# jeya-maria-jose/Medical-Transformer

Measured on AMD Instinct MI355X. Metric: training images/sec (MedT, 3x128x128), higher is better.
Workload: dtype f32; 1 GPU; MedT imgsize=128 bs=4/GPU train step (fwd+CE+bwd+Adam), BASELINE.json configs[2] (per GPU: also configs[3]'s shard); global_batch=4, parallelism=dp1

## Files before the change

medical-transformer_amd/csrc/conv.hip:

```cpp
#include "defer.h"
#include <type_traits>

namespace medt {

template <int K, int OT>
__device__ __forceinline__ void conv2d_fwd_body(
    const float* __restrict__ x, const float* __restrict__ w, const float* __restrict__ bias, float* __restrict__ y,
    float* __restrict__ partials, int Cin, int H, int W, int Cout, int Ho, int Wo, int stride, int pad, int relu,
    int npg, int y_bf16, float* red, int bx, int by) {
    constexpr int KK = K * K;
    const int HoWo = Ho * Wo, per_group = npg * HoWo, ppg = (per_group + MEDT_THREADS - 1) / MEDT_THREADS;
    const int grp = bx / ppg, part = bx - grp * ppg, o0 = by * OT;
    const int q = part * MEDT_THREADS + threadIdx.x;
    const bool ok = q < per_group;
    const int ni = ok ? q / HoWo : 0, p = ok ? q - ni * HoWo : 0;
    const int n = grp * npg + ni;
    const int ho = p / Wo, wo = p - ho * Wo;
    const int h0 = ho * stride - pad, w0 = wo * stride - pad;
    float acc[OT];
#pragma unroll
    for (int o = 0; o < OT; ++o) acc[o] = bias ? bias[o0 + o] : 0.f;
    const float* xn = x + (size_t)n * Cin * H * W;
    int off[KK];
#pragma unroll
// ... 676 lines not shown
            rb[i] = b;
        }
    };
    if (q_begin < q_end) fetch(q_begin);
    for (long q0 = q_begin; q0 < q_end; q0 += 64) {
#pragma unroll
        for (int i = 0; i < NA; ++i) A[r0 + 4 * i][j] = ra[i];
#pragma unroll
        for (int i = 0; i < NB; ++i) B[r0 + 4 * i][j] = rb[i];
        __syncthreads();
        if (q0 + 64 < q_end) fetch(q0 + 64);
#pragma unroll 2
        for (int jj = 0; jj < 64; jj += 4) {
            float4 av[RO], bv[RC];
#pragma unroll
            for (int a = 0; a < RO; ++a) av[a] = *reinterpret_cast<const float4*>(&A[to + 16 * a][jj]);
#pragma unroll
            for (int b = 0; b < RC; ++b) bv[b] = *reinterpret_cast<const float4*>(&B[tc + 16 * b][jj]);
#pragma unroll
            for (int a = 0; a < RO; ++a)
#pragma unroll
                for (int b = 0; b < RC; ++b) {
                    float t = acc[a][b];
                    t = fmaf(av[a].x, bv[b].x, t);
                    t = fmaf(av[a].y, bv[b].y, t);
                    t = fmaf(av[a].z, bv[b].z, t);
                    t = fmaf(av[a].w, bv[b].w, t);
                    acc[a][b] = t;
                }
        }
        __syncthreads();
    }
    float* out = scratch + (size_t)bz * Cout * Ktot;
#pragma unroll
    for (int a = 0; a < RO; ++a)
#pragma unroll
        for (int b = 0; b < RC; ++b) {
            const int o = o0 + to + 16 * a, k = k0 + tc + 16 * b;
            if (o < Cout && k < Ktot) out[(size_t)o * Ktot + k] = acc[a][b];
        }
}

template <int K, int TO, int TC>
__global__ __launch_bounds__(MEDT_THREADS) void conv_wgrad_kernel(
    const float* __restrict__ dy, const float* __restrict__ raw, const float* __restrict__ coef,
    const float* __restrict__ x, float* __restrict__ scratch, int N, int Cin, int H, int W, int Cout, int Ho, int Wo,
    int stride, int pad, int QS, int npg) {
    conv_wgrad_body<K, TO, TC>(dy, raw, coef, x, scratch, N, Cin, H, W, Cout, Ho, Wo, stride, pad, QS, npg, blockIdx.x,
                               blockIdx.y, blockIdx.z);
}

static inline int wgrad_tile(int n) { return n <= 16 ? 16 : (n <= 32 ? 32 : 64); }

static int wgrad_chunk(int Cout, int Ktot, long NP) {
    const long tiles = (long)cdiv(Cout, wgrad_tile(Cout)) * cdiv(Ktot, wgrad_tile(Ktot));
    int QS = 512;
    while (QS > 64 && tiles * ((NP + QS - 1) / QS) < 512) QS >>= 1;
    while ((NP + QS - 1) / QS > 64) QS <<= 1;
    return QS;
}

static int wgrad_chunk_grouped(long NP) {
    static const int target = 64;
    static const int qmax = 256;
    int QS = 64;
    while (QS < qmax && (NP + QS - 1) / QS > target) QS <<= 1;
    static const int smax = 64;
    static const int smax_big = 256;
    while ((NP + QS - 1) / QS > (NP >= 65536 ? smax_big : smax)) QS <<= 1;
    return QS;
}

static int wgrad_chunk_v4(long NP) {
    static const int target = 16;
    static const int qmax = 1024;
    static const int smax_big = 256;
    int QS = 256;
    while (QS < qmax && (NP + QS - 1) / QS > (NP >= 65536 ? smax_big : target)) QS <<= 1;
    while ((NP + QS - 1) / QS > (NP >= 65536 ? smax_big : 64)) QS <<= 1;
    const int QG = wgrad_chunk_grouped(NP);
    return QS > QG ? QS : QG;
}

int conv2d_bwd_weight_splits(int N, int Cin, int Cout, int K, int Ho, int Wo) {
    const long NP = (long)N * Ho * Wo;
    const int QS = wgrad_chunk(Cout, Cin * K * K, NP), QG = wgrad_chunk_grouped(NP);
    const int a = (int)((NP + QS - 1) / QS), b = (int)((NP + QG - 1) / QG);
    return a > b ? a : b;
}

int conv2d_bwd_weight(const float* dy, const float* raw, const float* coef, const float* x, float* dw, float* scratch,
                      int N, int Cin, int H, int W, int Cout, int K, int stride, int pad, int groups, hipStream_t s,
                      Queue* q) {
    const int Ho = (H + 2 * pad - K) / stride + 1, Wo = (W + 2 * pad - K) / stride + 1;
    const long NP = (long)N * Ho * Wo;
    const int Ktot = Cin * K * K;
    const bool mfma = conv_use_mfma(Cin, Cout, K, stride, NP) && Cout >= 64;
    const bool v4 = q && !mfma && conv_wgrad_v4_ok(dy, raw, x, N, Cin, H, W, Cout, Ho, Wo, K, stride, pad);
    const int QS = v4 ? wgrad_chunk_v4(NP) : ((q && !mfma) ? wgrad_chunk_grouped(NP) : wgrad_chunk(Cout, Ktot, NP));
    const int splits = (int)((NP + QS - 1) / QS);
    const dim3 grid(cdiv(Cout, 64), cdiv(Ktot, 64), splits), block(MEDT_THREADS);
    if (splits == 1) scratch = dw;
    if (mfma) {
        static const bool defer_m = true;
        if (q && defer_m) {
            q->mwgrad.push_back(MJob{dy, raw, coef, x, scratch, N, Cin, H, W, Cout, Ho, Wo, K, stride, pad, QS, splits, N / groups});
            if (splits > 1) q->reduce.push_back(RJob{scratch, dw, splits, Cout * Ktot});
            return MEDT_OK;
        }
        int rc = conv_wgrad_mfma(dy, raw, coef, x, scratch, N, Cin, H, W, Cout, Ho, Wo, K, stride, pad, QS, splits,
                                 N / groups, s);
        if (rc) return rc;
        if (splits == 1) return MEDT_OK;
        if (q) { q->reduce.push_back(RJob{scratch, dw, splits, Cout * Ktot}); return MEDT_OK; }
        return reduce_rows(scratch, splits, Cout * Ktot, dw, s);
    }
    if (q) {
        if (K != 1 && K != 3 && K != 7) { set_error("conv2d: kernel size %d unsupported (1, 3, 7)", K); return MEDT_EUNSUPPORTED; }
        q->wgrad.push_back(WJob{dy, raw, coef, x, scratch, N, Cin, H, W, Cout, Ho, Wo, stride, pad, QS, N / groups,
                                cdiv(Cout, 64), cdiv(Ktot, 64), splits, K, v4 ? 1 : 0});
        if (splits > 1) q->reduce.push_back(RJob{scratch, dw, splits, Cout * Ktot});
        return MEDT_OK;
    }
    {
        const int TO = wgrad_tile(Cout), TC = wgrad_tile(Ktot);
        const dim3 g2(cdiv(Cout, TO), cdiv(Ktot, TC), splits);
#define MEDT_WG(KV, TOV, TCV)                                                                                        \
    hipLaunchKernelGGL((conv_wgrad_kernel<KV, TOV, TCV>), g2, block, 0, s, dy, raw, coef, x, scratch, N, Cin, H, W, Cout, Ho, \
                       Wo, stride, pad, QS, N / groups)
#define MEDT_WG_TC(KV, TOV)                                                                                          \
    do { if (TC == 16) MEDT_WG(KV, TOV, 16); else if (TC == 32) MEDT_WG(KV, TOV, 32); else MEDT_WG(KV, TOV, 64); } while (0)
#define MEDT_WG_TO(KV)                                                                                               \
    do { if (TO == 16) MEDT_WG_TC(KV, 16); else if (TO == 32) MEDT_WG_TC(KV, 32); else MEDT_WG_TC(KV, 64); } while (0)
        switch (K) {
            case 1: MEDT_WG_TO(1); break;
            case 3: MEDT_WG_TO(3); break;
            case 7: MEDT_WG_TO(7); break;
            default: set_error("conv2d: kernel size %d unsupported (1, 3, 7)", K); return MEDT_EUNSUPPORTED;
        }
#undef MEDT_WG_TO
#undef MEDT_WG_TC
#undef MEDT_WG
    }
    int rc = launch_status("conv_wgrad");
    if (rc) return rc;
    return splits == 1 ? MEDT_OK : reduce_rows(scratch, splits, Cout * Ktot, dw, s);
}

#define CS_SPLITS 16
int channel_sum_splits_for(int N, int HW) {
    const long total = (long)N * HW;
    long sp = (total + 4095) / 4096;
    return sp < 1 ? 1 : (sp > CS_SPLITS ? CS_SPLITS : (int)sp);
}
__device__ __forceinline__ void channel_sum_body(const float* __restrict__ x, float* __restrict__ part, int N, int C,
                                                 int HW, int c, int sp, int splits) {
    MEDT_STATIC_SHARED float red[MEDT_WAVES];
    float v[1] = {0.f};
    const long total = (long)N * HW;
    const long per = (total + splits - 1) / splits, beg = sp * per, end = beg + per < total ? beg + per : total;
    if (total < (1l << 31)) {
        const unsigned e32 = (unsigned)end, hw = (unsigned)HW;
        float a4[4] = {0.f, 0.f, 0.f, 0.f};
        for (unsigned q = (unsigned)beg + threadIdx.x; q < e32; q += 4 * MEDT_THREADS) {
            float t[4];
#pragma unroll
            for (int u = 0; u < 4; ++u) {
                const unsigned qq = min(q + u * MEDT_THREADS, e32 - 1), n = qq / hw, p = qq - n * hw;
                t[u] = x[((size_t)n * C + c) * HW + p];
            }
#pragma unroll
            for (int u = 0; u < 4; ++u)
                if (q + u * MEDT_THREADS < e32) a4[u] += t[u];
        }
        v[0] = (a4[0] + a4[1]) + (a4[2] + a4[3]);
    } else {
        for (long q = beg + threadIdx.x; q < end; q += MEDT_THREADS) {
            const int n = (int)(q / HW), p = (int)(q - (long)n * HW);
            v[0] += x[((size_t)n * C + c) * HW + p];
        }
    }
    block_sum<1>(v, red, part + (size_t)sp * C + c);
}

__global__ __launch_bounds__(MEDT_THREADS) void channel_sum_kernel(const float* __restrict__ x, float* __restrict__ part,
                                                                   int N, int C, int HW) {
// ... 38 lines not shown
```

medical-transformer_amd/csrc/conv_mfma.hip:

```cpp
#include "defer.h"
#include <algorithm>
#include <vector>
#include <stdlib.h>
#include <stdio.h>

namespace medt {

typedef medt_f4 f32x4;

bool conv_use_mfma(int Cin, int Cout, int K, int stride, long positions) {
    static const bool off = [] { const char* e = getenv("MEDT_DISABLE_MFMA"); return e && e[0] == '1'; }();
    static const bool force = false;
    if (force && !off) return (K == 1 || K == 3) && (stride == 1 || stride == 2);
    const long tiles = ((positions + 63) / 64) * ((Cout + 63) / 64);
    if (off || Cout < 32 || Cin * K * K < 256 || (stride != 1 && stride != 2)) return false;
    if (K == 3 && tiles >= 128) return true;
    static const long few_pos = 2048L;
    return (K == 3 || K == 1) && tiles < 128 && positions <= few_pos && Cin * K * K >= 512;
}

int conv_mfma_parts_per_group(int N, int groups, int HoWo) { return cdiv((N / groups) * HoWo, 64); }

template <int K>
__global__ __launch_bounds__(MEDT_THREADS) void conv_mfma_fwd_kernel(
// ... 627 lines not shown
            if (o < Cout) {
                const float bo = a.bias ? a.bias[o] : 0.f;
                const size_t e0 = ((size_t)n * Cout + o) * HW + (size_t)row0 * W + col;
#pragma unroll
                for (int t = 0; t < TR; ++t) {
                    float v = acc[rb][t][r] + bo;
                    if (a.add) v += a.add[e0 + (size_t)t * W];
                    s1[r] += v;
                    s2[r] = fmaf(v, v, s2[r]);
                    a.y[e0 + (size_t)t * W] = a.relu ? fmaxf(v, 0.f) : v;
                }
            }
        }
        if (a.partials) {
#pragma unroll
            for (int r = 0; r < 4; ++r) {
                double pa = s1[r], pb = s2[r];
#pragma unroll
                for (int m = 8; m > 0; m >>= 1) { pa += __shfl_xor(pa, m, 64); pb += __shfl_xor(pb, m, 64); }
                if ((lane & 15) == 0) {
                    double* d = Rd + ((wv * NRB + rb) * 16 + (lane >> 4) * 4 + r) * 2;
                    d[0] = pa; d[1] = pb;
                }
            }
        }
    }
    if (a.partials) {
        __syncthreads();
        if (kg == 0 && tid < 16 * NRB) {
            const int o = o0 + tid;
            if (o < Cout) {
                double sa = 0.0, sb = 0.0;
#pragma unroll
                for (int w4 = 0; w4 < 4; ++w4) { sa += Rd[(w4 * 16 * NRB + tid) * 2]; sb += Rd[(w4 * 16 * NRB + tid) * 2 + 1]; }
                double* dst = reinterpret_cast<double*>(a.partials) + ((size_t)blockIdx.x * Cout + o) * 2;
                dst[0] = sa;
                dst[1] = sb;
            }
        }
    }
}

int conv_thin_fwd(const float* x, const float* w, const float* bias, const float* add, float* y, float* partials, int N, int groups,
                  int Cin, int H, int W, int Cout, int relu, hipStream_t s) {
    const ThinPlan p = conv_thin_plan(N, groups, Cin, H, W, Cout, 3, 1, 1);
    if (!p.ok) { set_error("conv_thin_fwd: shape not supported"); return MEDT_EUNSUPPORTED; }
    if (abl_skip("conv_thin")) return MEDT_OK;
    ThinArgs a;
    a.x = x; a.w = w; a.bias = bias; a.add = add; a.y = y; a.partials = partials;
    a.Cin = Cin; a.H = H; a.W = W; a.Cout = Cout; a.relu = relu;
    a.TCW = p.TCW; a.RG = p.RG; a.RST = p.RST; a.CST = p.CST; a.PR = p.rows_wg + 2; a.PC = p.cols_wg + 2; a.cwg = W / p.cols_wg;
    a.m_pc = (unsigned)(0x100000000ull / (unsigned)a.PC) + 1u;
    a.m_prpc = (unsigned)(0x100000000ull / (unsigned)(a.PR * a.PC)) + 1u;
    const dim3 grid((unsigned)(N * p.wgs_img), (unsigned)p.grid_y), block(MEDT_THREADS * p.KG);
#define MEDT_THIN(CCv, NRBv, TRv, KGv) hipLaunchKernelGGL((conv3x3_thin_fwd_kernel<CCv, NRBv, TRv, KGv>), grid, block, p.lds, s, a)
#define MEDT_THIN_TR(CCv, NRBv)                         \
    do {                                                \
        if (p.TR == 4) MEDT_THIN(CCv, NRBv, 4, 1);      \
        else if (p.TR == 2) MEDT_THIN(CCv, NRBv, 2, 1); \
        else MEDT_THIN(CCv, NRBv, 1, 1);                \
    } while (0)
    if (p.KG > 1) {
        static unsigned char attr[4][64];
        int rc;
        if ((rc = lds_opt_in((const void*)conv3x3_thin_fwd_kernel<16, 1, 1, 4>, attr[0], "conv3x3_thin_fwd")) ||
            (rc = lds_opt_in((const void*)conv3x3_thin_fwd_kernel<16, 2, 1, 4>, attr[1], "conv3x3_thin_fwd")) ||
            (rc = lds_opt_in((const void*)conv3x3_thin_fwd_kernel<16, 1, 1, 2>, attr[2], "conv3x3_thin_fwd")) ||
            (rc = lds_opt_in((const void*)conv3x3_thin_fwd_kernel<16, 2, 1, 2>, attr[3], "conv3x3_thin_fwd"))) return rc;
        if (p.NRB == 2) { if (p.KG == 4) MEDT_THIN(16, 2, 1, 4); else MEDT_THIN(16, 2, 1, 2); }
        else { if (p.KG == 4) MEDT_THIN(16, 1, 1, 4); else MEDT_THIN(16, 1, 1, 2); }
    }
    else if (p.CC == 16 && p.NRB == 2) MEDT_THIN_TR(16, 2);
    else if (p.CC == 16) MEDT_THIN_TR(16, 1);
    else if (p.NRB == 2) MEDT_THIN_TR(8, 2);
    else MEDT_THIN_TR(8, 1);
#undef MEDT_THIN_TR
#undef MEDT_THIN
    return launch_status("conv3x3_thin_fwd");
}

struct R16WJob {
    const float *dy, *raw, *coef, *x;
    float* scratch;
    int Cin, H, Cout, tiles_per_split, ptiles, npg, gx, gy, gz;
};

template <int OT>
__device__ __forceinline__ void conv3x3_rows16_wgrad_body(const R16WJob& jb, int bx, int by, int bz, float* Ds, float* Ps) {
    constexpr int NR = OT / 4;
    constexpr int NA = OT == 64 ? 9 : 5;
    const float* __restrict__ dy = jb.dy;
    const float* __restrict__ raw = jb.raw;
    const float* __restrict__ coef = jb.coef;
    const float* __restrict__ x = jb.x;
    float* __restrict__ scratch = jb.scratch;
    const int Cin = jb.Cin, H = jb.H, Cout = jb.Cout, tiles_per_split = jb.tiles_per_split, ptiles = jb.ptiles, npg = jb.npg;
    const int tid = threadIdx.x, lane = tid & 63, wv = __builtin_amdgcn_readfirstlane(tid >> 6);
    const int rb = OT == 64 ? wv : (wv & 1), tlo = OT == 64 ? 0 : 5 * (wv >> 1);
    const int o0 = bx * OT, c0 = by * 16;
    const int Ktot = Cin * 9, HW = H * 16, tpi = H >> 2;
    const int pt_begin = bz * tiles_per_split;
    const int pt_end = min(ptiles, pt_begin + tiles_per_split);
    if (tid < 192) {
        const int c = tid / 12, rem = tid - c * 12;
        Ps[c * R16_WCST + (rem >> 1) * R16_RST + (rem & 1) * 17] = 0.f;
    }
    int poff[6], pc[6], prw[6];
#pragma unroll
    for (int i = 0; i < 6; ++i) {
        const int u = tid + MEDT_THREADS * i, c = u / 96, rem = u - c * 96, row = rem >> 4, col = rem & 15;
        poff[i] = c * R16_WCST + row * R16_RST + 1 + col;
        pc[i] = (c0 + c) * HW + col;
        prw[i] = row - 1;
    }
    float rd[NR], rp[6];
    auto fetch = [&](int pt) {
        const int n = pt / tpi, r0 = (pt - n * tpi) * 4;
        const size_t base = (size_t)n * Cout * HW + r0 * 16 + lane;
        const float* cf = coef ? coef + (size_t)(n / npg) * Cout * 3 : nullptr;
#pragma unroll
        for (int j = 0; j < NR; ++j)
            rd[j] = dy[base + (size_t)min(o0 + wv + 4 * j, Cout - 1) * HW];
        if (cf) {
#pragma unroll
            for (int j = 0; j < NR; ++j) {
                const int o = min(o0 + wv + 4 * j, Cout - 1);
                rd[j] = fmaf(cf[o * 3], rd[j], fmaf(cf[o * 3 + 1], raw[base + (size_t)o * HW], cf[o * 3 + 2]));
            }
        }
        const float* xn = x + (size_t)n * Cin * HW;
#pragma unroll
        for (int i = 0; i < 6; ++i) {
            const int gr = r0 + prw[i];
            const float v = xn[pc[i] + min(max(gr, 0), H - 1) * 16];
            rp[i] = (unsigned)gr < (unsigned)H ? v : 0.f;
        }
    };
    f32x4 acc[NA];
#pragma unroll
    for (int t = 0; t < NA; ++t) acc[t] = (f32x4)(0.f);
    int tapoff[NA];
    float tapon[NA];
#pragma unroll
    for (int tt = 0; tt < NA; ++tt) {
        const int t = min(tlo + tt, 8);
        tapoff[tt] = (t / 3) * R16_RST + t % 3;
        tapon[tt] = tlo + tt <= 8 ? 1.f : 0.f;
    }
    const float* drow = Ds + (16 * rb + (lane & 15)) * R16_DST + (lane >> 4);
    const float* prow = Ps + (lane & 15) * R16_WCST + (lane >> 4);
    if (pt_begin < pt_end) fetch(pt_begin);
    for (int pt = pt_begin; pt < pt_end; ++pt) {
#pragma unroll
        for (int j = 0; j < NR; ++j) Ds[(wv + 4 * j) * R16_DST + lane] = rd[j];
#pragma unroll
        for (int i = 0; i < 6; ++i) Ps[poff[i]] = rp[i];
        __syncthreads();
        if (pt + 1 < pt_end) fetch(pt + 1);
#pragma unroll
        for (int ks = 0; ks < 16; ++ks) {
            const float a = drow[ks * 4];
            const float* pk = prow + (ks >> 2) * R16_RST + (ks & 3) * 4;
#pragma unroll
            for (int tt = 0; tt < NA; ++tt)
                acc[tt] = __builtin_amdgcn_mfma_f32_16x16x4f32(OT == 64 ? a : a * tapon[tt], pk[tapoff[tt]], acc[tt], 0, 0, 0);
        }
        __syncthreads();
    }
    float* out = scratch + (size_t)bz * Cout * Ktot;
#pragma unroll
    for (int r = 0; r < 4; ++r) {
        const int o = o0 + 16 * rb + (lane >> 4) * 4 + r;
        if (o < Cout) {
            float* dst = out + (size_t)o * Ktot + (c0 + (lane & 15)) * 9;
#pragma unroll
            for (int tt = 0; tt < NA; ++tt)
                if (tlo + tt <= 8) dst[tlo + tt] = acc[tt][r];
        }
    }
}

using R16WBatch = JobBatch<R16WJob, 4>;
template <int OT>
__global__ __launch_bounds__(MEDT_THREADS) void conv3x3_rows16_wgrad_kernel(R16WBatch b) {
    MEDT_STATIC_SHARED float Ds[OT * R16_DST];
    MEDT_STATIC_SHARED float Ps[16 * R16_WCST];
    const int j = find_job(b, blockIdx.x);
    const R16WJob& jb = b.job[j];
    const int r = blockIdx.x - b.start[j], bx = r % jb.gx, by = (r / jb.gx) % jb.gy, bz = r / (jb.gx * jb.gy);
    conv3x3_rows16_wgrad_body<OT>(jb, bx, by, bz, Ds, Ps);
}

__global__ __launch_bounds__(MEDT_THREADS) void conv_splitk_epilogue_kernel(
    const float* __restrict__ slices, int nslices, size_t slice_stride, const float* __restrict__ bias,
    float* __restrict__ y, float* __restrict__ partials, int Cout, int HoWo, int npg, int ppg64, int relu) {
    MEDT_STATIC_SHARED float red[MEDT_WAVES * 2 * 2];
    const int per_group = npg * HoWo, ppg = (per_group + MEDT_THREADS - 1) / MEDT_THREADS;
    const int grp = blockIdx.x / ppg, part = blockIdx.x - grp * ppg, o = blockIdx.y;
    const int q = part * MEDT_THREADS + threadIdx.x;
    float v[2] = {0.f, 0.f};
    if (q < per_group) {
        const size_t qg = (size_t)grp * ppg64 * 64 + q;
        float a = bias ? bias[o] : 0.f;
        const float* sp = slices + qg * Cout + o;
        int s = 0;
        for (; s + 8 <= nslices; s += 8) {
            float v[8];
#pragma unroll
            for (int u = 0; u < 8; ++u) v[u] = sp[(size_t)(s + u) * slice_stride];
            MEDT_SCHED_FENCE();
#pragma unroll
            for (int u = 0; u < 8; ++u) a += v[u];
            MEDT_SCHED_FENCE();
        }
        for (; s < nslices; ++s) a += sp[(size_t)s * slice_stride];
        const int n = grp * npg + q / HoWo, p = q % HoWo;
        y[((size_t)n * Cout + o) * HoWo + p] = relu ? fmaxf(a, 0.f) : a;
        v[0] = a;
        v[1] = a * a;
    }
    if (partials) block_sum_d<2>(v, red, reinterpret_cast<double*>(partials) + ((size_t)blockIdx.x * Cout + o) * 2);
}

int conv_mfma_ksplit(int Ktot, long tiles, bool rows16) {
#ifdef MEDT_AB_KSPLIT128
    if (tiles >= 128) return 1;
#else
    if (tiles >= 256 || (rows16 && tiles >= 128)) return 1;
    if (tiles >= 128) return Ktot >= 256 ? 2 : 1;
#endif
    int ks = (int)(256 / tiles);
    const int maxks = Ktot / 64 > 0 ? Ktot / 64 : 1;
    if (ks > maxks) ks = maxks;
    return ks < 1 ? 1 : ks;
}

size_t conv_mfma_scratch_floats(int N, int groups, int HoWo, int Cin, int Cout, int K, bool rows16) {
    const long qt = (long)groups * conv_mfma_parts_per_group(N, groups, HoWo);
    const int ks = conv_mfma_ksplit(Cin * K * K, qt * cdiv(Cout, 64), rows16);
    return ks > 1 ? (size_t)ks * qt * 64 * Cout : 0;
}

int conv_mfma_fwd(const float* x, const float* w, const float* bias, float* y, float* partials, float* scratch, int N,
                  int Cin, int H, int W, int Cout, int K, int stride, int pad, int relu, int groups, hipStream_t s) {
    const int Ho = (H + 2 * pad - K) / stride + 1, Wo = (W + 2 * pad - K) / stride + 1;
    const int ppg64 = conv_mfma_parts_per_group(N, groups, Ho * Wo), Ktot = Cin * K * K;
    const long qt = (long)groups * ppg64;
    int ks = scratch ? conv_mfma_ksplit(Ktot, qt * cdiv(Cout, 64), conv_rows16_ok(Cin, H, W, K, stride, pad)) : 1;
    int kchunk = Ktot;
    if (ks > 1) {
        kchunk = cdiv(cdiv(Ktot, ks), 16) * 16;
        ks = cdiv(Ktot, kchunk);
    }
    const dim3 grid((unsigned)qt, cdiv(Cout, 64), ks), block(MEDT_THREADS);
    if (ks == 1 && (N / groups) * Ho * Wo % 64 == 0 && conv_rows16_ok(Cin, H, W, K, stride, pad)) {
        if (abl_skip("rows16")) return MEDT_OK;
        static const int force_ot = [] { const char* e = getenv("MEDT_R16_OT"); return e ? atoi(e) : 0; }();
        const bool half = force_ot == 32 || (force_ot != 64 && qt * cdiv(Cout, 64) < 768);
        if (half)
            hipLaunchKernelGGL(conv3x3_rows16_fwd_kernel<32>, dim3((unsigned)qt, cdiv(Cout, 32)), block, 0, s, x, w, bias, y,
                               partials, Cin, H, Cout, relu);
        else
            hipLaunchKernelGGL(conv3x3_rows16_fwd_kernel<64>, dim3((unsigned)qt, cdiv(Cout, 64)), block, 0, s, x, w, bias, y,
                               partials, Cin, H, Cout, relu);
        return launch_status("conv3x3_rows16_fwd");
    }
    float* kout = ks > 1 ? scratch : nullptr;
    if (K == 1)
        hipLaunchKernelGGL(conv_mfma_fwd_kernel<1>, grid, block, 0, s, x, w, bias, y, partials, Cin, H, W, Cout, Ho, Wo,
                           stride, pad, relu, N / groups, kchunk, kout);
    else
        hipLaunchKernelGGL(conv_mfma_fwd_kernel<3>, grid, block, 0, s, x, w, bias, y, partials, Cin, H, W, Cout, Ho, Wo,
                           stride, pad, relu, N / groups, kchunk, kout);
// ... 452 lines not shown
};
using WBatch = JobBatch<WJobP, 42>;
static_assert(sizeof(WBatch) <= 4000, "job table must fit the kernel-argument block");
template <int TO>
__global__ __launch_bounds__(MEDT_THREADS, 3) void conv_wgrad_mfma_grouped_kernel(WBatch b) {
    MEDT_STATIC_SHARED __attribute__((aligned(16))) float smem[(TO == 32 ? 96 * V4_LD : (TO + 64) * 65)];
    float (*A)[65] = reinterpret_cast<float (*)[65]>(smem);
    float (*B)[65] = reinterpret_cast<float (*)[65]>(smem + TO * 65);
    const int j = find_job(b, blockIdx.x);
    const WJobP& w = b.job[j];
    const int local = blockIdx.x - b.start[j];
    const int gx = (w.Cout + TO - 1) / TO, gy = (w.Cin * w.K * w.K + 63) / 64;
    const int bx = local % gx, t = local / gx, by = t % gy, bz = t / gy;
    if constexpr (TO == 32) {
        if (w.v4) {
            if (w.K == 1) conv_wgrad_v4_body32<1>(w.dy, w.raw, w.coef, w.x, w.scratch, w.N, w.Cin, w.H * w.W, w.W, w.Cout, w.QS, w.npg, bx, by, bz, smem);
            else conv_wgrad_v4_body32<3>(w.dy, w.raw, w.coef, w.x, w.scratch, w.N, w.Cin, w.H * w.W, w.W, w.Cout, w.QS, w.npg, bx, by, bz, smem);
            return;
        }
    }
#define MEDT_WG_BODY(KV)                                                                                                 \
    do {                                                                                                                 \
        if constexpr (TO == 64)                                                                                          \
            conv_wgrad_mfma_body<KV>(w.dy, w.raw, w.coef, w.x, w.scratch, w.N, w.Cin, w.H, w.W, w.Cout, w.Ho, w.Wo,      \
                                     w.stride, w.pad, w.QS, w.npg, bx, by, bz, A, B);                                    \
        else                                                                                                             \
            conv_wgrad_mfma_body32<KV>(w.dy, w.raw, w.coef, w.x, w.scratch, w.N, w.Cin, w.H, w.W, w.Cout, w.Ho, w.Wo,    \
                                       w.stride, w.pad, w.QS, w.npg, bx, by, bz, A, B);                                  \
    } while (0)
    if (w.K == 1) MEDT_WG_BODY(1);
    else if (w.K == 3) MEDT_WG_BODY(3);
    else MEDT_WG_BODY(7);
#undef MEDT_WG_BODY
}

bool conv_wgrad_v4_ok(const float* dy, const float* raw, const float* x, int N, int Cin, int H, int W, int Cout, int Ho, int Wo,
                      int K, int stride, int pad) {
    if (stride != 1 || Ho != H || Wo != W) return false;
    if (!((K == 1 && pad == 0 && (H * W) % 4 == 0) || (K == 3 && pad == 1 && W % 4 == 0))) return false;
    if ((((uintptr_t)dy | (uintptr_t)raw | (uintptr_t)x) & 15) != 0) return false;
    const size_t HW = (size_t)H * W;
    return (size_t)N * Cout * HW * 4 < 0xffffffffull && (size_t)N * Cin * HW * 4 < 0xffffffffull;
}

int conv_wgrad_grouped(const WJob* jobs, int n, hipStream_t s) {
    constexpr int to = 32;
    std::vector<int> order(n);
    for (int j = 0; j < n; ++j) order[j] = j;
    auto cost = [&](int j) { return (long)((jobs[j].QS + 63) / 64) * (jobs[j].K == 1 ? 2 : 3); };
    std::stable_sort(order.begin(), order.end(), [&](int a, int b) { return cost(a) > cost(b); });
    WBatch b;
    b.n = 0;
    int blocks = 0;
    auto launch = [&]() -> int {
        b.start[b.n] = blocks;
#ifdef MEDT_ABLATE
        if (getenv("MEDT_WG_DEBUG")) {
            fprintf(stderr, "wgrad grouped: %d jobs, %d blocks\n", b.n, blocks);
            for (int j = 0; j < b.n; ++j) {
                const WJobP& w = b.job[j];
                fprintf(stderr, "  wjob K%d v4 %d Cout %3d Cin %3d HoWo %3dx%3d N %2d QS %4d blocks %4d (o-tiles %d k-tiles %d chunks %d)\n", (int)w.K, (int)w.v4,
                        w.Cout, w.Cin, w.Ho, w.Wo, w.N, w.QS, b.start[j + 1] - b.start[j], (w.Cout + 31) / 32, (w.Cin * w.K * w.K + 63) / 64, w.gz);
            }
        }
#endif
        hipLaunchKernelGGL(conv_wgrad_mfma_grouped_kernel<32>, dim3(blocks), dim3(MEDT_THREADS), 0, s, b);
        b.n = 0;
        blocks = 0;
        return launch_status("conv_wgrad_mfma_grouped");
    };
    for (int i = 0; i < n; ++i) {
        const WJob& w = jobs[order[i]];
        if (w.K != 1 && w.K != 3 && w.K != 7) { set_error("conv2d: kernel size %d unsupported (1, 3, 7)", w.K); return MEDT_EUNSUPPORTED; }
        b.job[b.n] = WJobP{w.dy, w.raw, w.coef, w.x, w.scratch, w.N, w.Cin, w.H, w.W, w.Cout, w.Ho, w.Wo, w.QS, w.npg, w.gz,
                           (unsigned char)w.stride, (unsigned char)w.pad, (unsigned char)w.K, (unsigned char)(to == 32 && w.v4)};
        b.start[b.n] = blocks;
        blocks += cdiv(w.Cout, to) * w.gy * w.gz;
        if (++b.n == 42) { int rc = launch(); if (rc) return rc; }
    }
    if (b.n) { int rc = launch(); if (rc) return rc; }
    return MEDT_OK;
}

bool conv_wgrad_rows16_ok(int Cin, int H, int W, int Ho, int Wo, int K, int stride, int pad, int QS) {
    return QS % 64 == 0 && Ho == H && Wo == W && conv_rows16_ok(Cin, H, W, K, stride, pad);
}

int conv_wgrad_rows16_grouped(const MJob* const* jobs, int n, hipStream_t s) {
    if (abl_skip(jobs[0]->N >= 16 ? "wgrad_mfma_l" : "wgrad_mfma_g")) return MEDT_OK;
    static const int ot = 64;
    for (int i0 = 0; i0 < n; i0 += 4) {
        R16WBatch b;
        b.n = n - i0 < 4 ? n - i0 : 4;
        int blocks = 0;
        for (int i = 0; i < b.n; ++i) {
            const MJob& m = *jobs[i0 + i];
            R16WJob& j = b.job[i];
            j.dy = m.dy; j.raw = m.raw; j.coef = m.coef; j.x = m.x; j.scratch = m.scratch;
            j.Cin = m.Cin; j.H = m.H; j.Cout = m.Cout; j.tiles_per_split = m.QS / 64; j.ptiles = m.N * m.H / 4; j.npg = m.npg;
            j.gx = cdiv(m.Cout, ot); j.gy = m.Cin / 16; j.gz = m.splits;
            b.start[i] = blocks;
            blocks += j.gx * j.gy * j.gz;
        }
        b.start[b.n] = blocks;
        if (ot == 32) hipLaunchKernelGGL(conv3x3_rows16_wgrad_kernel<32>, dim3(blocks), dim3(MEDT_THREADS), 0, s, b);
        else hipLaunchKernelGGL(conv3x3_rows16_wgrad_kernel<64>, dim3(blocks), dim3(MEDT_THREADS), 0, s, b);
        int rc = launch_status("conv3x3_rows16_wgrad");
        if (rc) return rc;
    }
    return MEDT_OK;
}

int conv_wgrad_mfma(const float* dy, const float* raw, const float* coef, const float* x, float* scratch, int N, int Cin,
                    int H, int W, int Cout, int Ho, int Wo, int K, int stride, int pad, int QS, int splits, int npg,
                    hipStream_t s) {
    const dim3 grid(cdiv(Cout, 64), cdiv(Cin * K * K, 64), splits), block(MEDT_THREADS);
    if (abl_skip(N >= 16 ? "wgrad_mfma_l" : "wgrad_mfma_g")) return MEDT_OK;
    if (conv_wgrad_rows16_ok(Cin, H, W, Ho, Wo, K, stride, pad, QS)) {
        const MJob m{dy, raw, coef, x, scratch, N, Cin, H, W, Cout, Ho, Wo, K, stride, pad, QS, splits, npg};
        const MJob* one = &m;
        return conv_wgrad_rows16_grouped(&one, 1, s);
    }
    if (K == 1)
        hipLaunchKernelGGL(conv_wgrad_mfma_kernel<1>, grid, block, 0, s, dy, raw, coef, x, scratch, N, Cin, H, W, Cout, Ho,
                           Wo, stride, pad, QS, npg);
    else
        hipLaunchKernelGGL(conv_wgrad_mfma_kernel<3>, grid, block, 0, s, dy, raw, coef, x, scratch, N, Cin, H, W, Cout, Ho,
                           Wo, stride, pad, QS, npg);
    return launch_status("conv_wgrad_mfma");
}

}
```

medical-transformer_amd/csrc/defer.h:

```cpp
#pragma once
#include "medt_kernels.h"
#include <vector>

namespace medt {

struct BnFin {
    const float* partials;
    int ppg, CH;
    double count;
    const float *weight, *bias;
    float *running_mean, *running_var;
    int64_t* nbt;
    BnStats out;
};
struct FinJob { BnFin f; int groups, training; float momentum, eps; };
struct BfinJob {
    const float* partials;
    int ppg, groups, CH, training;
    double count;
    float dscale;
    BnStats st;
    const float* weight;
    float *coef, *dweight, *dbias;
};
struct SmallFinArgs {
    const float *part_ob, *part_sb, *part_qb;
    BnStats so, ss, sq;
    float *d_out_w, *d_out_b, *d_sim_w, *d_sim_b, *d_qkv_w, *d_qkv_b;
    int C, G, groups, training;
    double row_count, sim_count;
    float dscale_out;
};
struct RJob { const float* src; float* dst; int P, K; };
struct FlipJob { const float* w; float* wt; int Cout, Cin, K; };
struct CJob { const float* x; float* part; int N, C, HW, splits; };
struct WJob {
    const float *dy, *raw, *coef, *x;
    float* scratch;
    int N, Cin, H, W, Cout, Ho, Wo, stride, pad, QS, npg, gx, gy, gz, K;
    int v4;
};

struct MJob {
    const float *dy, *raw, *coef, *x;
    float* scratch;
    int N, Cin, H, W, Cout, Ho, Wo, K, stride, pad, QS, splits, npg;
};

struct RelfixJob {
    const float *relative, *sim_coef, *pg_part, *gate_raw;
    BnStats ss;
    GatePtrs gates;
    float *rel_rows, *gate_rows;
    double sim_count;
    int L, G, SC, hq, nparts, sweep_gridx, training, blocks;
    unsigned lds;
    float eps;
    BfinJob qb;
    int qb_on, qb_nch;
};

struct Queue {
    std::vector<FinJob> fin;
    std::vector<BfinJob> bfin;
    std::vector<SmallFinArgs> sfin;
    std::vector<CJob> csum;
    std::vector<WJob> wgrad;
    std::vector<MJob> mwgrad;
    std::vector<RJob> reduce;
    std::vector<FlipJob> flip;
    size_t pending() const {
        return flip.size() + fin.size() + bfin.size() + sfin.size() + csum.size() + wgrad.size() + mwgrad.size() + reduce.size();
    }
};

Queue* queue_for(hipStream_t s);

BnFin make_fin(const float* partials, int ppg, int CH, double count, const medt_bn_ptrs& bn, BnStats out);

int conv_flip_weights_grouped(const FlipJob* jobs, int n, hipStream_t s);
int bn_finalize_grouped(const FinJob* jobs, int n, hipStream_t s);
int bn_bwd_finalize_grouped(const BfinJob* jobs, int n, hipStream_t s);
int wopos_small_bwd_finalize_grouped(const SmallFinArgs* jobs, int n, hipStream_t s);
int reduce_rows_grouped(const RJob* jobs, int n, hipStream_t s);
int channel_sum_grouped(const CJob* jobs, int n, hipStream_t s);
int conv_wgrad_grouped(const WJob* jobs, int n, hipStream_t s);
bool conv_wgrad_v4_ok(const float* dy, const float* raw, const float* x, int N, int Cin, int H, int W, int Cout, int Ho, int Wo,
                      int K, int stride, int pad);
bool conv_wgrad_rows16_ok(int Cin, int H, int W, int Ho, int Wo, int K, int stride, int pad, int QS);
int conv_wgrad_rows16_grouped(const MJob* const* jobs, int n, hipStream_t s);
int conv_wgrad_mfma_batch(const MJob* const* jobs, int n, hipStream_t s);

template <class J, int MAXJ>
struct JobBatch {
    int n;
    int start[MAXJ + 1];
    J job[MAXJ];
};
template <class B>
__device__ __forceinline__ int find_job(const B& b, int block) {
    int lo = 0, hi = b.n;
    while (hi - lo > 1) {
        const int mid = (lo + hi) >> 1;
        if (block >= b.start[mid]) lo = mid; else hi = mid;
    }
    return lo;
}

}
```

Baseline: 2185 images/s.

## Route non-MFMA 3x3 conv weight-grads through generalized rows16 MFMA patch kernel

Extends the rows16 MFMA weight-gradient kernel to widths that are multiples of 16 by tiling over column patches and loading halo columns. Small 3x3 stride-1 convolutions that previously used the scalar v4/grouped wgrad path now go through the deferred MFMA batch. It also adds 16- and 32-wide output tiles chosen per job, enlarges the job batch to 40 entries, and sorts jobs by cost. The cost is extra halo loads, more split scratch, and a fixed s_nop delay before the epilogue.

```diff
diff --git a/medical-transformer_amd/csrc/conv.hip b/medical-transformer_amd/csrc/conv.hip
--- a/medical-transformer_amd/csrc/conv.hip
+++ b/medical-transformer_amd/csrc/conv.hip
@@ -782,11 +782,21 @@
     return QS > QG ? QS : QG;
 }
 
+static int wgrad_chunk_patch(long NP) {
+#ifdef MEDT_AB_PATCH_QS512
+    static const int qmin = 512;
+#else
+    static const int qmin = 256;
+#endif
+    const int QG = wgrad_chunk_grouped(NP);
+    return QG > qmin ? QG : qmin;
+}
+
 int conv2d_bwd_weight_splits(int N, int Cin, int Cout, int K, int Ho, int Wo) {
     const long NP = (long)N * Ho * Wo;
-    const int QS = wgrad_chunk(Cout, Cin * K * K, NP), QG = wgrad_chunk_grouped(NP);
-    const int a = (int)((NP + QS - 1) / QS), b = (int)((NP + QG - 1) / QG);
-    return a > b ? a : b;
+    const int QS = wgrad_chunk(Cout, Cin * K * K, NP), QG = wgrad_chunk_grouped(NP), QP = wgrad_chunk_patch(NP);
+    const int a = (int)((NP + QS - 1) / QS), b = (int)((NP + QG - 1) / QG), p = (int)((NP + QP - 1) / QP);
+    return std::max(a, std::max(b, p));
 }
 
 int conv2d_bwd_weight(const float* dy, const float* raw, const float* coef, const float* x, float* dw, float* scratch,
@@ -796,12 +806,15 @@
     const long NP = (long)N * Ho * Wo;
     const int Ktot = Cin * K * K;
     const bool mfma = conv_use_mfma(Cin, Cout, K, stride, NP) && Cout >= 64;
-    const bool v4 = q && !mfma && conv_wgrad_v4_ok(dy, raw, x, N, Cin, H, W, Cout, Ho, Wo, K, stride, pad);
-    const int QS = v4 ? wgrad_chunk_v4(NP) : ((q && !mfma) ? wgrad_chunk_grouped(NP) : wgrad_chunk(Cout, Ktot, NP));
+    const bool patch = !mfma && Ho == H && Wo == W && conv_wgrad_patch_shape_ok(Cin, H, W, K, stride, pad) &&
+                       conv_wgrad_rows16_ok(Cin, H, W, Ho, Wo, K, stride, pad, wgrad_chunk_patch(NP));
+    const bool v4 = q && !mfma && !patch && conv_wgrad_v4_ok(dy, raw, x, N, Cin, H, W, Cout, Ho, Wo, K, stride, pad);
+    const int QS = patch ? wgrad_chunk_patch(NP)
+                         : (v4 ? wgrad_chunk_v4(NP) : ((q && !mfma) ? wgrad_chunk_grouped(NP) : wgrad_chunk(Cout, Ktot, NP)));
     const int splits = (int)((NP + QS - 1) / QS);
     const dim3 grid(cdiv(Cout, 64), cdiv(Ktot, 64), splits), block(MEDT_THREADS);
     if (splits == 1) scratch = dw;
-    if (mfma) {
+    if (mfma || patch) {
         static const bool defer_m = true;
         if (q && defer_m) {
             q->mwgrad.push_back(MJob{dy, raw, coef, x, scratch, N, Cin, H, W, Cout, Ho, Wo, K, stride, pad, QS, splits, N / groups});
diff --git a/medical-transformer_amd/csrc/conv_mfma.hip b/medical-transformer_amd/csrc/conv_mfma.hip
--- a/medical-transformer_amd/csrc/conv_mfma.hip
+++ b/medical-transformer_amd/csrc/conv_mfma.hip
@@ -733,41 +733,43 @@
 struct R16WJob {
     const float *dy, *raw, *coef, *x;
     float* scratch;
-    int Cin, H, Cout, tiles_per_split, ptiles, npg, gx, gy, gz;
+    int Cin, H, W, Cout, tiles_per_split, ptiles, npg, gx, gy, gz, ot;
 };
 
 template <int OT>
 __device__ __forceinline__ void conv3x3_rows16_wgrad_body(const R16WJob& jb, int bx, int by, int bz, float* Ds, float* Ps) {
     constexpr int NR = OT / 4;
-    constexpr int NA = OT == 64 ? 9 : 5;
+    constexpr int NA = OT == 64 ? 9 : (OT == 32 ? 5 : 3);
     const float* __restrict__ dy = jb.dy;
     const float* __restrict__ raw = jb.raw;
     const float* __restrict__ coef = jb.coef;
     const float* __restrict__ x = jb.x;
     float* __restrict__ scratch = jb.scratch;
-    const int Cin = jb.Cin, H = jb.H, Cout = jb.Cout, tiles_per_split = jb.tiles_per_split, ptiles = jb.ptiles, npg = jb.npg;
+    const int Cin = jb.Cin, H = jb.H, W = jb.W, Cout = jb.Cout, tiles_per_split = jb.tiles_per_split, ptiles = jb.ptiles, npg = jb.npg;
     const int tid = threadIdx.x, lane = tid & 63, wv = __builtin_amdgcn_readfirstlane(tid >> 6);
-    const int rb = OT == 64 ? wv : (wv & 1), tlo = OT == 64 ? 0 : 5 * (wv >> 1);
+    const int rb = OT == 64 ? wv : (OT == 32 ? (wv & 1) : 0);
+    const int tlo = OT == 64 ? 0 : (OT == 32 ? 5 * (wv >> 1) : (wv ? 1 + 2 * wv : 0));
+    const int ntap = OT == 64 ? 9 : (OT == 32 ? 5 - (wv >> 1) : (wv ? 2 : 3));
     const int o0 = bx * OT, c0 = by * 16;
-    const int Ktot = Cin * 9, HW = H * 16, tpi = H >> 2;
+    const int Ktot = Cin * 9, HW = H * W, ctiles = W >> 4, tpi = (H >> 2) * ctiles;
     const int pt_begin = bz * tiles_per_split;
     const int pt_end = min(ptiles, pt_begin + tiles_per_split);
-    if (tid < 192) {
-        const int c = tid / 12, rem = tid - c * 12;
-        Ps[c * R16_WCST + (rem >> 1) * R16_RST + (rem & 1) * 17] = 0.f;
-    }
     int poff[6], pc[6], prw[6];
 #pragma unroll
     for (int i = 0; i < 6; ++i) {
         const int u = tid + MEDT_THREADS * i, c = u / 96, rem = u - c * 96, row = rem >> 4, col = rem & 15;
         poff[i] = c * R16_WCST + row * R16_RST + 1 + col;
-        pc[i] = (c0 + c) * HW + col;
+        pc[i] = min(c0 + c, Cin - 1) * HW + col;
         prw[i] = row - 1;
     }
-    float rd[NR], rp[6];
+    const int hcw = min(tid, 191) / 12, hrem = min(tid, 191) - hcw * 12, hside = hrem & 1;
+    const int hoff = hcw * R16_WCST + (hrem >> 1) * R16_RST + hside * 17;
+    const int hc = min(c0 + hcw, Cin - 1) * HW, hrw = (hrem >> 1) - 1;
+    const int dpos = (lane >> 4) * W + (lane & 15);
+    float rd[NR], rp[6], rh = 0.f;
     auto fetch = [&](int pt) {
-        const int n = pt / tpi, r0 = (pt - n * tpi) * 4;
-        const size_t base = (size_t)n * Cout * HW + r0 * 16 + lane;
+        const int n = pt / tpi, t = pt - n * tpi, band = t / ctiles, r0 = band * 4, col0 = (t - band * ctiles) * 16;
+        const size_t base = (size_t)n * Cout * HW + r0 * W + col0 + dpos;
         const float* cf = coef ? coef + (size_t)(n / npg) * Cout * 3 : nullptr;
 #pragma unroll
         for (int j = 0; j < NR; ++j)
@@ -779,12 +781,17 @@
                 rd[j] = fmaf(cf[o * 3], rd[j], fmaf(cf[o * 3 + 1], raw[base + (size_t)o * HW], cf[o * 3 + 2]));
             }
         }
-        const float* xn = x + (size_t)n * Cin * HW;
+        const float* xn = x + (size_t)n * Cin * HW + col0;
 #pragma unroll
         for (int i = 0; i < 6; ++i) {
             const int gr = r0 + prw[i];
-            const float v = xn[pc[i] + min(max(gr, 0), H - 1) * 16];
+            const float v = xn[pc[i] + min(max(gr, 0), H - 1) * W];
             rp[i] = (unsigned)gr < (unsigned)H ? v : 0.f;
+        }
+        if (ctiles > 1 && tid < 192) {
+            const int gr = r0 + hrw, gc = col0 + (hside ? 16 : -1);
+            const float v = x[(size_t)n * Cin * HW + hc + min(max(gr, 0), H - 1) * W + min(max(gc, 0), W - 1)];
+            rh = ((unsigned)gr < (unsigned)H && (unsigned)gc < (unsigned)W) ? v : 0.f;
         }
     };
     f32x4 acc[NA];
@@ -796,7 +803,7 @@
     for (int tt = 0; tt < NA; ++tt) {
         const int t = min(tlo + tt, 8);
         tapoff[tt] = (t / 3) * R16_RST + t % 3;
-        tapon[tt] = tlo + tt <= 8 ? 1.f : 0.f;
+        tapon[tt] = tt < ntap ? 1.f : 0.f;
     }
     const float* drow = Ds + (16 * rb + (lane & 15)) * R16_DST + (lane >> 4);
     const float* prow = Ps + (lane & 15) * R16_WCST + (lane >> 4);
@@ -806,6 +813,7 @@
         for (int j = 0; j < NR; ++j) Ds[(wv + 4 * j) * R16_DST + lane] = rd[j];
 #pragma unroll
         for (int i = 0; i < 6; ++i) Ps[poff[i]] = rp[i];
+        if (tid < 192) Ps[hoff] = rh;
         __syncthreads();
         if (pt + 1 < pt_end) fetch(pt + 1);
 #pragma unroll
@@ -818,28 +826,39 @@
         }
         __syncthreads();
     }
+#ifndef MEDT_LANE_EMU
+    MEDT_SCHED_FENCE();
+    asm volatile("s_nop 15\n\ts_nop 15" ::: "memory");
+    MEDT_SCHED_FENCE();
+#endif
     float* out = scratch + (size_t)bz * Cout * Ktot;
+    const int c = c0 + (lane & 15);
 #pragma unroll
     for (int r = 0; r < 4; ++r) {
         const int o = o0 + 16 * rb + (lane >> 4) * 4 + r;
-        if (o < Cout) {
-            float* dst = out + (size_t)o * Ktot + (c0 + (lane & 15)) * 9;
+        if (o < Cout && c < Cin) {
+            float* dst = out + (size_t)o * Ktot + c * 9;
 #pragma unroll
             for (int tt = 0; tt < NA; ++tt)
-                if (tlo + tt <= 8) dst[tlo + tt] = acc[tt][r];
-        }
-    }
-}
-
-using R16WBatch = JobBatch<R16WJob, 4>;
-template <int OT>
-__global__ __launch_bounds__(MEDT_THREADS) void conv3x3_rows16_wgrad_kernel(R16WBatch b) {
-    MEDT_STATIC_SHARED float Ds[OT * R16_DST];
+                if (tt < ntap) dst[tlo + tt] = acc[tt][r];
+        }
+    }
+}
+
+using R16WBatch = JobBatch<R16WJob, 40>;
+static_assert(sizeof(R16WBatch) <= 4000, "job table must fit the kernel-argument block");
+template <int MAXOT>
+__global__ __launch_bounds__(MEDT_THREADS, MAXOT == 64 ? 1 : 5) void conv3x3_rows16_wgrad_kernel(R16WBatch b) {
+    MEDT_STATIC_SHARED float Ds[MAXOT * R16_DST];
     MEDT_STATIC_SHARED float Ps[16 * R16_WCST];
     const int j = find_job(b, blockIdx.x);
     const R16WJob& jb = b.job[j];
     const int r = blockIdx.x - b.start[j], bx = r % jb.gx, by = (r / jb.gx) % jb.gy, bz = r / (jb.gx * jb.gy);
-    conv3x3_rows16_wgrad_body<OT>(jb, bx, by, bz, Ds, Ps);
+    if constexpr (MAXOT == 64) {
+        if (jb.ot == 64) { conv3x3_rows16_wgrad_body<64>(jb, bx, by, bz, Ds, Ps); return; }
+    }
+    if (jb.ot == 32) conv3x3_rows16_wgrad_body<32>(jb, bx, by, bz, Ds, Ps);
+    else conv3x3_rows16_wgrad_body<16>(jb, bx, by, bz, Ds, Ps);
 }
 
 __global__ __launch_bounds__(MEDT_THREADS) void conv_splitk_epilogue_kernel(
@@ -1458,29 +1477,51 @@
     return MEDT_OK;
 }
 
+bool conv_wgrad_patch_shape_ok(int Cin, int H, int W, int K, int stride, int pad) {
+    static const bool off = [] { const char* e = getenv("MEDT_WGRAD_PATCH"); return e && e[0] == '0'; }();
+    return !off && K == 3 && stride == 1 && pad == 1 && W % 16 == 0 && H % 4 == 0 && Cin >= 8 &&
+           conv_rows16_ok(16, 4, 16, 3, 1, 1);
+}
+
 bool conv_wgrad_rows16_ok(int Cin, int H, int W, int Ho, int Wo, int K, int stride, int pad, int QS) {
-    return QS % 64 == 0 && Ho == H && Wo == W && conv_rows16_ok(Cin, H, W, K, stride, pad);
+    if (QS % 64 != 0 || Ho != H || Wo != W) return false;
+    if (conv_rows16_ok(Cin, H, W, K, stride, pad)) return true;
+    return QS <= 1024 && conv_wgrad_patch_shape_ok(Cin, H, W, K, stride, pad);
+}
+
+static int r16w_ot(int Cout, int Cin) {
+#ifdef MEDT_AB_PATCH_OT32
+    return Cout >= 64 && Cin >= 32 ? 64 : 32;
+#else
+    return Cout >= 64 && Cin >= 32 ? 64 : (Cout <= 16 ? 16 : 32);
+#endif
 }
 
 int conv_wgrad_rows16_grouped(const MJob* const* jobs, int n, hipStream_t s) {
     if (abl_skip(jobs[0]->N >= 16 ? "wgrad_mfma_l" : "wgrad_mfma_g")) return MEDT_OK;
-    static const int ot = 64;
-    for (int i0 = 0; i0 < n; i0 += 4) {
+    constexpr int maxj = (int)(sizeof(R16WBatch::job) / sizeof(R16WJob));
+    std::vector<int> order(n);
+    for (int j = 0; j < n; ++j) order[j] = j;
+    auto cost = [&](int j) { const int ot = r16w_ot(jobs[j]->Cout, jobs[j]->Cin); return (long)(jobs[j]->QS / 64) * (ot == 64 ? 9 : (ot == 32 ? 5 : 3)); };
+    std::stable_sort(order.begin(), order.end(), [&](int a, int b) { return cost(a) > cost(b); });
+    for (int i0 = 0; i0 < n; i0 += maxj) {
         R16WBatch b;
-        b.n = n - i0 < 4 ? n - i0 : 4;
-        int blocks = 0;
+        b.n = n - i0 < maxj ? n - i0 : maxj;
+        int blocks = 0, maxot = 0;
         for (int i = 0; i < b.n; ++i) {
-            const MJob& m = *jobs[i0 + i];
+            const MJob& m = *jobs[order[i0 + i]];
             R16WJob& j = b.job[i];
             j.dy = m.dy; j.raw = m.raw; j.coef = m.coef; j.x = m.x; j.scratch = m.scratch;
-            j.Cin = m.Cin; j.H = m.H; j.Cout = m.Cout; j.tiles_per_split = m.QS / 64; j.ptiles = m.N * m.H / 4; j.npg = m.npg;
-            j.gx = cdiv(m.Cout, ot); j.gy = m.Cin / 16; j.gz = m.splits;
+            j.Cin = m.Cin; j.H = m.H; j.W = m.W; j.Cout = m.Cout; j.tiles_per_split = m.QS / 64;
+            j.ptiles = m.N * (m.H / 4) * (m.W / 16); j.npg = m.npg; j.ot = r16w_ot(m.Cout, m.Cin);
+            j.gx = cdiv(m.Cout, j.ot); j.gy = cdiv(m.Cin, 16); j.gz = m.splits;
             b.start[i] = blocks;
             blocks += j.gx * j.gy * j.gz;
+            maxot = j.ot > maxot ? j.ot : maxot;
         }
         b.start[b.n] = blocks;
-        if (ot == 32) hipLaunchKernelGGL(conv3x3_rows16_wgrad_kernel<32>, dim3(blocks), dim3(MEDT_THREADS), 0, s, b);
-        else hipLaunchKernelGGL(conv3x3_rows16_wgrad_kernel<64>, dim3(blocks), dim3(MEDT_THREADS), 0, s, b);
+        if (maxot == 64) hipLaunchKernelGGL(conv3x3_rows16_wgrad_kernel<64>, dim3(blocks), dim3(MEDT_THREADS), 0, s, b);
+        else hipLaunchKernelGGL(conv3x3_rows16_wgrad_kernel<32>, dim3(blocks), dim3(MEDT_THREADS), 0, s, b);
         int rc = launch_status("conv3x3_rows16_wgrad");
         if (rc) return rc;
     }
diff --git a/medical-transformer_amd/csrc/defer.h b/medical-transformer_amd/csrc/defer.h
--- a/medical-transformer_amd/csrc/defer.h
+++ b/medical-transformer_amd/csrc/defer.h
@@ -88,6 +88,7 @@
 bool conv_wgrad_v4_ok(const float* dy, const float* raw, const float* x, int N, int Cin, int H, int W, int Cout, int Ho, int Wo,
                       int K, int stride, int pad);
 bool conv_wgrad_rows16_ok(int Cin, int H, int W, int Ho, int Wo, int K, int stride, int pad, int QS);
+bool conv_wgrad_patch_shape_ok(int Cin, int H, int W, int K, int stride, int pad);
 int conv_wgrad_rows16_grouped(const MJob* const* jobs, int n, hipStream_t s);
 int conv_wgrad_mfma_batch(const MJob* const* jobs, int n, hipStream_t s);
 
```

Result: no change. 2190 images/s, median of 2 (+0.2%).
